# OpenDriveLab/ThinkTwice

Hardware: AMD Instinct MI355X
Metric: frames/sec forward (4-cam+LiDAR, thinktwice.py cfg) (higher is better)
Workload: dtype bf16x3h; 1 GPU; forward_inference thinktwice.py cfg: 8 frames x (2 sweeps x 4 cams x 448x896 + 65536-pt LiDAR), ResNet50+PAFPN+DepthNet+UNet+LSS splat, LidarNet, fusion, 5-stage decoder; parallelism=replicas x1 (no data-path collective), launch=eager launches, 3 batches in flight on alternating streams, batches_in_flight=3

## Files before the change

### include/thinktwice_hip.h

```cpp
#ifndef THINKTWICE_HIP_H
#define THINKTWICE_HIP_H

#include <stddef.h>
#include <stdint.h>

#ifdef __cplusplus
extern "C" {
#endif

#define TT_F32 0
#define TT_BF16 1
#define TT_F16 2

#define TT_ACT_NONE 0
#define TT_ACT_RELU 1
#define TT_ACT_SIGMOID 2
#define TT_ACT_GELU 3
#define TT_ACT_SOFTPLUS 4
#define TT_ACT_SOFTPLUS_CLAMP 5

const char* tt_last_error(void);
const char* tt_conv_last_kernel(void);
int tt_conv_set_trace(void* stamps_or_null);
int tt_version(void);
// ... 124 lines not shown
int tt_mlp_chain_wide_set_max_spin(int polls);
int tt_mlp_chain_wide_set_trace(void* stamps_or_null);

long long tt_dec_gru_scratch_floats(int B);
int tt_dec_gru(int B, const float* inp6, const float* state, float* fut, float* scratch, const void* const* w0,
               const float* const* wx, const float* const* b0, const void* const* w2, const float* const* b2,
               const void* wd0, const float* bd0, const void* wd2, const float* bd2, void* stream);
long long tt_dec_flatten_scratch_floats(int maps);
int tt_dec_flatten(int maps, const float* in, float* out, float* mids_or_null, float* scratch, const void* const* w,
                   const float* const* b, const float* bn_scale, const float* bn_shift, void* stream);
int tt_dec_set_trace(void* stamps_or_null);
long long tt_dec_bev_update_scratch_floats(int B);
int tt_dec_bev_update(int B, const float* bev, const float* G, float* out, long long out_bstride, float* out2,
                      long long out2_bstride, float* scratch, const void* w0, const float* b0, const void* const* w2,
                      const float* b2, void* stream);

int tt_nchw_to_nhwc_pad(const float* in, void* out, int N, int C, int H, int W, int Cp,
                        int out_dtype, void* stream);
int tt_nchw_to_nhwc_border(const float* in, void* out, int N, int C, int H, int W, int Cp, int Hp, int Wp,
                           int top, int left, int out_dtype, void* stream);
int tt_nhwc_to_nchw(const void* in, float* out, int N, int C, int H, int W, int cstride, int coff,
                    int in_dtype, void* stream);
int tt_maxpool3x3s2(const void* in, void* out, int N, int H, int W, int C, int dtype, void* stream);
int tt_upsample_nearest_add(void* dst, const void* src, int N, int H, int W, int C, int h, int w,
                            int dtype, void* stream);
int tt_bilinear_up2(const void* in, void* out, int N, int H, int W, int C, int dtype, void* stream);
int tt_bilinear_up2_pair(const float* in, float* out, int N, int H, int W, int C, void* stream);
int tt_spatial_pool(const void* in, float* out, int N, int HW, int C, int cstride, int coff, int mode,
                    int dtype, void* stream);
int tt_channel_gate(const void* x, const float* gate, const void* res, void* out, int N, int HW, int C,
                    int gate_act, int out_act, int dtype, void* stream);
int tt_affine_rows(const void* x, const float* scale, const float* shift, void* out, long long R, int C,
                   int x_stride, int out_stride, int act, int dtype, void* stream);
int tt_layernorm_rows(const void* x, const float* gamma, const float* beta, void* out, long long R,
                      int D, int x_stride, int out_stride, float eps, int dtype, void* stream);
int tt_copy_nhwc(const void* in, void* out, int N, int H, int W, int C, int in_cstride, int in_coff,
                 int out_cstride, int out_coff, int rot_flip, int in_dtype, int out_dtype, void* stream);
int tt_broadcast_rows(const void* v, void* out, int N, int HW, int C, int v_stride, int out_cstride,
                      int out_coff, int dtype, void* stream);
int tt_ew(const void* a, const void* b, const void* g, void* out, long long R, int C, int a_stride,
          int a_coff, int b_stride, int b_coff, int g_stride, int g_coff, int o_stride, int o_coff,
          int op, int act, int dtype, void* stream);
int tt_concat_rows(float* out, long long R, int out_stride, int nseg, const float* const* srcs, const int* strides,
                   const int* widths, const int* coffs, const int* divs, const int* mods, void* stream);

int tt_deform_im2col3x3(const void* x, const float* offsets, void* cols, int N, int H, int W, int C,
// ... 415 lines not shown
```

### thinktwice_amd/build.py

```python
import os
import subprocess
import sys
from concurrent.futures import ThreadPoolExecutor

from . import _lib

HERE = os.path.dirname(os.path.abspath(__file__))
CSRC = os.path.join(HERE, "csrc")
OBJ = os.path.join(CSRC, "_obj")
LIB = os.path.join(HERE, "libthinktwice_hip.so")
HIPCC = os.environ.get("HIPCC", "/opt/rocm/bin/hipcc")
FLAGS = ["--offload-arch=gfx950", "-O3", "-std=c++17", "-fPIC", "-munsafe-fp-atomics", "-ffp-contract=off",
         "-Wno-unused-result"]


EXTRA_FLAGS = {"conv_x3_pipe.hip": ["-fno-slp-vectorize"], "conv_x3_up2.hip": ["-fno-slp-vectorize"],
               "conv_x3_patch.hip": ["-fno-slp-vectorize"], "conv_x3_join.hip": ["-fno-slp-vectorize"]}


def _sources():
    return sorted(f for f in os.listdir(CSRC) if f.endswith((".hip", ".cpp")))


def _deps_mtime():
    hdrs = [os.path.join(CSRC, f) for f in os.listdir(CSRC) if f.endswith((".h", ".inc"))]
    hdrs.append(os.path.join(HERE, "..", "include", "thinktwice_hip.h"))
    hdrs.append(os.path.abspath(__file__))
    return max(os.path.getmtime(h) for h in hdrs)


def _compile(src, hdr_mtime, verbose):
    obj = os.path.join(OBJ, src + ".o")
    spath = os.path.join(CSRC, src)
    if os.path.exists(obj) and os.path.getmtime(obj) > max(os.path.getmtime(spath), hdr_mtime):
        return obj
    cmd = [HIPCC] + FLAGS + EXTRA_FLAGS.get(src, []) + (["-x", "hip"] if src.endswith(".hip") else []) + ["-c", spath, "-o", obj]
    if verbose:
        print(" ".join(cmd), flush=True)
    subprocess.run(cmd, check=True)
    return obj
# ... 73 lines not shown
```

### thinktwice_amd/csrc/plan_thunks.inc

```

static int thunk_tt_voxel_pool_fwd(const PlanVal* a, void* stream) { return tt_voxel_pool_fwd((int)a[0].i, (int)a[1].i, (int)a[2].i, (int)a[3].i, (int)a[4].i, (int)a[5].i, (const int32_t*)a[6].p, (const float*)a[7].p, (float*)a[8].p, (int32_t*)a[9].p, stream); }
static int thunk_tt_voxel_pool_fwd_ws(const PlanVal* a, void* stream) { return tt_voxel_pool_fwd_ws((int)a[0].i, (int)a[1].i, (int)a[2].i, (int)a[3].i, (int)a[4].i, (int)a[5].i, (const int32_t*)a[6].p, (const float*)a[7].p, (float*)a[8].p, (int32_t*)a[9].p, (void*)a[10].p, (long long)a[11].i, stream); }
static int thunk_tt_voxel_pool_plan_build(const PlanVal* a, void* stream) { return tt_voxel_pool_plan_build((int)a[0].i, (int)a[1].i, (int)a[2].i, (int)a[3].i, (int)a[4].i, (const int32_t*)a[5].p, (void*)a[6].p, (long long)a[7].i, (void*)a[8].p, (long long)a[9].i, stream); }
static int thunk_tt_voxel_pool_fwd_planned(const PlanVal* a, void* stream) { return tt_voxel_pool_fwd_planned((int)a[0].i, (int)a[1].i, (int)a[2].i, (int)a[3].i, (int)a[4].i, (const void*)a[5].p, (const float*)a[6].p, (float*)a[7].p, (void*)a[8].p, (long long)a[9].i, stream); }
static int thunk_tt_voxel_pool_bwd(const PlanVal* a, void* stream) { return tt_voxel_pool_bwd((int)a[0].i, (int)a[1].i, (int)a[2].i, (int)a[3].i, (int)a[4].i, (const int32_t*)a[5].p, (const float*)a[6].p, (float*)a[7].p, stream); }
static int thunk_tt_frustum_voxel_index(const PlanVal* a, void* stream) { return tt_frustum_voxel_index((int)a[0].i, (int)a[1].i, (int)a[2].i, (int)a[3].i, (int)a[4].i, (const float*)a[5].p, (const float*)a[6].p, (const float*)a[7].p, (const float*)a[8].p, (int32_t*)a[9].p, (float*)a[10].p, stream); }
static int thunk_tt_lift_splat_fwd(const PlanVal* a, void* stream) { return tt_lift_splat_fwd((int)a[0].i, (int)a[1].i, (int)a[2].i, (int)a[3].i, (int)a[4].i, (int)a[5].i, (int)a[6].i, (int)a[7].i, (int)a[8].i, (const void*)a[9].p, (const void*)a[10].p, (int)a[11].i, (const int32_t*)a[12].p, (float*)a[13].p, (int)a[14].i, (int)a[15].i, (int)a[16].i, stream); }
static int thunk_tt_lift_splat_fwd_ws(const PlanVal* a, void* stream) { return tt_lift_splat_fwd_ws((int)a[0].i, (int)a[1].i, (int)a[2].i, (int)a[3].i, (int)a[4].i, (int)a[5].i, (int)a[6].i, (int)a[7].i, (int)a[8].i, (const void*)a[9].p, (const void*)a[10].p, (int)a[11].i, (const int32_t*)a[12].p, (float*)a[13].p, (int)a[14].i, (int)a[15].i, (int)a[16].i, (void*)a[17].p, (long long)a[18].i, stream); }
static int thunk_tt_conv2d_fwd(const PlanVal* a, void* stream) { return tt_conv2d_fwd((const tt_conv_desc*)a[0].p, stream); }
static int thunk_tt_conv2d_fwd_next(const PlanVal* a, void* stream) { return tt_conv2d_fwd_next((const tt_conv_desc*)a[0].p, (const tt_conv_next*)a[1].p, stream); }
static int thunk_tt_seg_feedback_chain(const PlanVal* a, void* stream) { return tt_seg_feedback_chain((const float*)a[0].p, (long long)a[1].i, (int)a[2].i, (int)a[3].i, (const float*)a[4].p, (const float*)a[5].p, (const float*)a[6].p, (int)a[7].i, (const float*)a[8].p, (const void*)a[9].p, (int)a[10].i, (const float*)a[11].p, (const float*)a[12].p, (int)a[13].i, (float*)a[14].p, (int)a[15].i, (int)a[16].i, stream); }
static int thunk_tt_mlp_chain(const PlanVal* a, void* stream) { return tt_mlp_chain((const float*)a[0].p, (long long)a[1].i, (int)a[2].i, (int)a[3].i, (const tt_chain_stage*)a[4].p, (int)a[5].i, stream); }
static int thunk_tt_mlp_chain_wide(const PlanVal* a, void* stream) { return tt_mlp_chain_wide((const float*)a[0].p, (long long)a[1].i, (int)a[2].i, (int)a[3].i, (const tt_chain_stage*)a[4].p, (int)a[5].i, (void*)a[6].p, (long long)a[7].i, stream); }
static int thunk_tt_dec_gru(const PlanVal* a, void* stream) { return tt_dec_gru((int)a[0].i, (const float*)a[1].p, (const float*)a[2].p, (float*)a[3].p, (float*)a[4].p, (const void* const*)a[5].p, (const float* const*)a[6].p, (const float* const*)a[7].p, (const void* const*)a[8].p, (const float* const*)a[9].p, (const void*)a[10].p, (const float*)a[11].p, (const void*)a[12].p, (const float*)a[13].p, stream); }
static int thunk_tt_dec_flatten(const PlanVal* a, void* stream) { return tt_dec_flatten((int)a[0].i, (const float*)a[1].p, (float*)a[2].p, (float*)a[3].p, (float*)a[4].p, (const void* const*)a[5].p, (const float* const*)a[6].p, (const float*)a[7].p, (const float*)a[8].p, stream); }
static int thunk_tt_dec_bev_update(const PlanVal* a, void* stream) { return tt_dec_bev_update((int)a[0].i, (const float*)a[1].p, (const float*)a[2].p, (float*)a[3].p, (long long)a[4].i, (float*)a[5].p, (long long)a[6].i, (float*)a[7].p, (const void*)a[8].p, (const float*)a[9].p, (const void* const*)a[10].p, (const float*)a[11].p, stream); }
static int thunk_tt_nchw_to_nhwc_pad(const PlanVal* a, void* stream) { return tt_nchw_to_nhwc_pad((const float*)a[0].p, (void*)a[1].p, (int)a[2].i, (int)a[3].i, (int)a[4].i, (int)a[5].i, (int)a[6].i, (int)a[7].i, stream); }
static int thunk_tt_nchw_to_nhwc_border(const PlanVal* a, void* stream) { return tt_nchw_to_nhwc_border((const float*)a[0].p, (void*)a[1].p, (int)a[2].i, (int)a[3].i, (int)a[4].i, (int)a[5].i, (int)a[6].i, (int)a[7].i, (int)a[8].i, (int)a[9].i, (int)a[10].i, (int)a[11].i, stream); }
static int thunk_tt_nhwc_to_nchw(const PlanVal* a, void* stream) { return tt_nhwc_to_nchw((const void*)a[0].p, (float*)a[1].p, (int)a[2].i, (int)a[3].i, (int)a[4].i, (int)a[5].i, (int)a[6].i, (int)a[7].i, (int)a[8].i, stream); }
static int thunk_tt_maxpool3x3s2(const PlanVal* a, void* stream) { return tt_maxpool3x3s2((const void*)a[0].p, (void*)a[1].p, (int)a[2].i, (int)a[3].i, (int)a[4].i, (int)a[5].i, (int)a[6].i, stream); }
static int thunk_tt_upsample_nearest_add(const PlanVal* a, void* stream) { return tt_upsample_nearest_add((void*)a[0].p, (const void*)a[1].p, (int)a[2].i, (int)a[3].i, (int)a[4].i, (int)a[5].i, (int)a[6].i, (int)a[7].i, (int)a[8].i, stream); }
static int thunk_tt_bilinear_up2(const PlanVal* a, void* stream) { return tt_bilinear_up2((const void*)a[0].p, (void*)a[1].p, (int)a[2].i, (int)a[3].i, (int)a[4].i, (int)a[5].i, (int)a[6].i, stream); }
static int thunk_tt_bilinear_up2_pair(const PlanVal* a, void* stream) { return tt_bilinear_up2_pair((const float*)a[0].p, (float*)a[1].p, (int)a[2].i, (int)a[3].i, (int)a[4].i, (int)a[5].i, stream); }
static int thunk_tt_spatial_pool(const PlanVal* a, void* stream) { return tt_spatial_pool((const void*)a[0].p, (float*)a[1].p, (int)a[2].i, (int)a[3].i, (int)a[4].i, (int)a[5].i, (int)a[6].i, (int)a[7].i, (int)a[8].i, stream); }
static int thunk_tt_channel_gate(const PlanVal* a, void* stream) { return tt_channel_gate((const void*)a[0].p, (const float*)a[1].p, (const void*)a[2].p, (void*)a[3].p, (int)a[4].i, (int)a[5].i, (int)a[6].i, (int)a[7].i, (int)a[8].i, (int)a[9].i, stream); }
static int thunk_tt_affine_rows(const PlanVal* a, void* stream) { return tt_affine_rows((const void*)a[0].p, (const float*)a[1].p, (const float*)a[2].p, (void*)a[3].p, (long long)a[4].i, (int)a[5].i, (int)a[6].i, (int)a[7].i, (int)a[8].i, (int)a[9].i, stream); }
static int thunk_tt_layernorm_rows(const PlanVal* a, void* stream) { return tt_layernorm_rows((const void*)a[0].p, (const float*)a[1].p, (const float*)a[2].p, (void*)a[3].p, (long long)a[4].i, (int)a[5].i, (int)a[6].i, (int)a[7].i, (float)a[8].d, (int)a[9].i, stream); }
static int thunk_tt_copy_nhwc(const PlanVal* a, void* stream) { return tt_copy_nhwc((const void*)a[0].p, (void*)a[1].p, (int)a[2].i, (int)a[3].i, (int)a[4].i, (int)a[5].i, (int)a[6].i, (int)a[7].i, (int)a[8].i, (int)a[9].i, (int)a[10].i, (int)a[11].i, (int)a[12].i, stream); }
static int thunk_tt_broadcast_rows(const PlanVal* a, void* stream) { return tt_broadcast_rows((const void*)a[0].p, (void*)a[1].p, (int)a[2].i, (int)a[3].i, (int)a[4].i, (int)a[5].i, (int)a[6].i, (int)a[7].i, (int)a[8].i, stream); }
static int thunk_tt_ew(const PlanVal* a, void* stream) { return tt_ew((const void*)a[0].p, (const void*)a[1].p, (const void*)a[2].p, (void*)a[3].p, (long long)a[4].i, (int)a[5].i, (int)a[6].i, (int)a[7].i, (int)a[8].i, (int)a[9].i, (int)a[10].i, (int)a[11].i, (int)a[12].i, (int)a[13].i, (int)a[14].i, (int)a[15].i, (int)a[16].i, stream); }
static int thunk_tt_concat_rows(const PlanVal* a, void* stream) { return tt_concat_rows((float*)a[0].p, (long long)a[1].i, (int)a[2].i, (int)a[3].i, (const float* const*)a[4].p, (const int*)a[5].p, (const int*)a[6].p, (const int*)a[7].p, (const int*)a[8].p, (const int*)a[9].p, stream); }
static int thunk_tt_deform_im2col3x3(const PlanVal* a, void* stream) { return tt_deform_im2col3x3((const void*)a[0].p, (const float*)a[1].p, (void*)a[2].p, (int)a[3].i, (int)a[4].i, (int)a[5].i, (int)a[6].i, (int)a[7].i, (int)a[8].i, (int)a[9].i, stream); }
static int thunk_tt_look_project_pack(const PlanVal* a, void* stream) { return tt_look_project_pack((int)a[0].i, (const float*)a[1].p, (const float*)a[2].p, (const float*)a[3].p, (float)a[4].d, (float)a[5].d, (float*)a[6].p, (int*)a[7].p, (int*)a[8].p, (int*)a[9].p, stream); }
static int thunk_tt_look_gather_query(const PlanVal* a, void* stream) { return tt_look_gather_query((int)a[0].i, (const int*)a[1].p, (const float*)a[2].p, (const float*)a[3].p, (const float*)a[4].p, (const float*)a[5].p, (const float*)a[6].p, (const float*)a[7].p, (const float*)a[8].p, (const void* const*)a[9].p, (const int*)a[10].p, (int)a[11].i, (float*)a[12].p, (int)a[13].i, stream); }
static int thunk_tt_msda_sample(const PlanVal* a, void* stream) { return tt_msda_sample((int)a[0].i, (const void*)a[1].p, (int)a[2].i, (const float*)a[3].p, (const float*)a[4].p, (const float*)a[5].p, (const int*)a[6].p, (float*)a[7].p, stream); }
static int thunk_tt_msda_sample_strided(const PlanVal* a, void* stream) { return tt_msda_sample_strided((int)a[0].i, (const void*)a[1].p, (int)a[2].i, (int)a[3].i, (int)a[4].i, (const float*)a[5].p, (const float*)a[6].p, (const float*)a[7].p, (const int*)a[8].p, (float*)a[9].p, stream); }
static int thunk_tt_sca_reduce(const PlanVal* a, void* stream) { return tt_sca_reduce((int)a[0].i, (const float*)a[1].p, (const int*)a[2].p, (float*)a[3].p, stream); }
static int thunk_tt_look_query_ln(const PlanVal* a, void* stream) { return tt_look_query_ln((int)a[0].i, (const int*)a[1].p, (const float*)a[2].p, (const float*)a[3].p, (const float*)a[4].p, (int)a[5].i, (const float*)a[6].p, (const float*)a[7].p, (const float*)a[8].p, (const float*)a[9].p, (const void* const*)a[10].p, (const int*)a[11].p, (int)a[12].i, (const float*)a[13].p, (const float*)a[14].p, (float)a[15].d, (float*)a[16].p, (int)a[17].i, stream); }
static int thunk_tt_msda_sample_ln(const PlanVal* a, void* stream) { return tt_msda_sample_ln((int)a[0].i, (const void*)a[1].p, (int)a[2].i, (int)a[3].i, (int)a[4].i, (const float*)a[5].p, (const float*)a[6].p, (const float*)a[7].p, (const int*)a[8].p, (const float*)a[9].p, (const float*)a[10].p, (float)a[11].d, (float*)a[12].p, (float*)a[13].p, (const int*)a[14].p, stream); }
static int thunk_tt_msda_sample_proj_ln(const PlanVal* a, void* stream) { return tt_msda_sample_proj_ln((int)a[0].i, (const void* const*)a[1].p, (const int*)a[2].p, (const float*)a[3].p, (const float*)a[4].p, (const float*)a[5].p, (const float*)a[6].p, (const float*)a[7].p, (const float*)a[8].p, (const float*)a[9].p, (const float*)a[10].p, (float)a[11].d, (float*)a[12].p, (float*)a[13].p, (const int*)a[14].p, stream); }
static int thunk_tt_sca_reduce_ln(const PlanVal* a, void* stream) { return tt_sca_reduce_ln((int)a[0].i, (const float*)a[1].p, (const int*)a[2].p, (const float*)a[3].p, (const float*)a[4].p, (float)a[5].d, (float*)a[6].p, stream); }
static int thunk_tt_dec_merge_in(const PlanVal* a, void* stream) { return tt_dec_merge_in((int)a[0].i, (const float*)a[1].p, (const float*)a[2].p, (const float*)a[3].p, (const float*)a[4].p, (const float*)a[5].p, (const float*)a[6].p, (float)a[7].d, (float*)a[8].p, stream); }
static int thunk_tt_lidar_voxelize(const PlanVal* a, void* stream) { return tt_lidar_voxelize((const float*)a[0].p, (int)a[1].i, (int)a[2].i, (int)a[3].i, (const float*)a[4].p, (const float*)a[5].p, (const int*)a[6].p, (int)a[7].i, (int)a[8].i, (void*)a[9].p, (long long)a[10].i, (float*)a[11].p, (int*)a[12].p, (int*)a[13].p, stream); }
// ... 65 lines not shown
static int thunk_tt_copy_bytes(const PlanVal* a, void* stream) { return tt_copy_bytes((void*)a[0].p, (const void*)a[1].p, (long long)a[2].i, stream); }

static const PlanThunk kPlanThunks[] = {
    {"tt_voxel_pool_fwd", thunk_tt_voxel_pool_fwd, 10},
    {"tt_voxel_pool_fwd_ws", thunk_tt_voxel_pool_fwd_ws, 12},
    {"tt_voxel_pool_plan_build", thunk_tt_voxel_pool_plan_build, 10},
    {"tt_voxel_pool_fwd_planned", thunk_tt_voxel_pool_fwd_planned, 10},
    {"tt_voxel_pool_bwd", thunk_tt_voxel_pool_bwd, 8},
    {"tt_frustum_voxel_index", thunk_tt_frustum_voxel_index, 11},
    {"tt_lift_splat_fwd", thunk_tt_lift_splat_fwd, 17},
    {"tt_lift_splat_fwd_ws", thunk_tt_lift_splat_fwd_ws, 19},
    {"tt_conv2d_fwd", thunk_tt_conv2d_fwd, 1},
    {"tt_conv2d_fwd_next", thunk_tt_conv2d_fwd_next, 2},
    {"tt_seg_feedback_chain", thunk_tt_seg_feedback_chain, 17},
    {"tt_mlp_chain", thunk_tt_mlp_chain, 6},
    {"tt_mlp_chain_wide", thunk_tt_mlp_chain_wide, 8},
    {"tt_dec_gru", thunk_tt_dec_gru, 14},
    {"tt_dec_flatten", thunk_tt_dec_flatten, 9},
    {"tt_dec_bev_update", thunk_tt_dec_bev_update, 12},
    {"tt_nchw_to_nhwc_pad", thunk_tt_nchw_to_nhwc_pad, 8},
    {"tt_nchw_to_nhwc_border", thunk_tt_nchw_to_nhwc_border, 12},
    {"tt_nhwc_to_nchw", thunk_tt_nhwc_to_nchw, 9},
    {"tt_maxpool3x3s2", thunk_tt_maxpool3x3s2, 7},
    {"tt_upsample_nearest_add", thunk_tt_upsample_nearest_add, 9},
    {"tt_bilinear_up2", thunk_tt_bilinear_up2, 7},
    {"tt_bilinear_up2_pair", thunk_tt_bilinear_up2_pair, 6},
    {"tt_spatial_pool", thunk_tt_spatial_pool, 9},
    {"tt_channel_gate", thunk_tt_channel_gate, 10},
    {"tt_affine_rows", thunk_tt_affine_rows, 10},
    {"tt_layernorm_rows", thunk_tt_layernorm_rows, 10},
    {"tt_copy_nhwc", thunk_tt_copy_nhwc, 13},
    {"tt_broadcast_rows", thunk_tt_broadcast_rows, 9},
    {"tt_ew", thunk_tt_ew, 17},
    {"tt_concat_rows", thunk_tt_concat_rows, 10},
    {"tt_deform_im2col3x3", thunk_tt_deform_im2col3x3, 10},
    {"tt_look_project_pack", thunk_tt_look_project_pack, 10},
    {"tt_look_gather_query", thunk_tt_look_gather_query, 14},
    {"tt_msda_sample", thunk_tt_msda_sample, 8},
    {"tt_msda_sample_strided", thunk_tt_msda_sample_strided, 10},
    {"tt_sca_reduce", thunk_tt_sca_reduce, 4},
    {"tt_look_query_ln", thunk_tt_look_query_ln, 18},
    {"tt_msda_sample_ln", thunk_tt_msda_sample_ln, 15},
    {"tt_msda_sample_proj_ln", thunk_tt_msda_sample_proj_ln, 15},
    {"tt_sca_reduce_ln", thunk_tt_sca_reduce_ln, 7},
    {"tt_dec_merge_in", thunk_tt_dec_merge_in, 9},
    {"tt_lidar_voxelize", thunk_tt_lidar_voxelize, 14},
// ... 68 lines not shown
```

### thinktwice_amd/lss.py

```python
import os

import torch

from . import _lib, camera, layers, ops, weights
from .layers import conv_from_sd, conv_from_weight, deconv2x2_from_sd, linear_from_sd, rows, unrows
from .registry import BACKBONES, NECKS, build_neck


class _ResNet50:

    def __init__(self, sd, p, dtype, device):
        vec = weights.vec_of(dtype)
        self.cin_pad = vec
        self.stem = conv_from_sd(sd, p + ".conv1", dtype, device, bn=p + ".bn1", stride=2, pad=3, act="relu",
                                 cin_pad=vec)
        self.stem_rr, self.stem_rr_x3 = None, None
        if weights.storage_dtype(dtype) != torch.float32:
            w = sd[p + ".conv1.weight"].to(device)
            wr = torch.zeros(w.shape[0], 7, 1, 64, dtype=dtype, device=device)
            wr[:, :, 0, :56] = torch.nn.functional.pad(w.permute(0, 2, 3, 1), (0, 5)).reshape(w.shape[0], 7, 56).to(dtype)
            self.stem_rr = wr.contiguous()
        elif dtype == weights.X3 and os.environ.get("TT_X3_STEM_ROWRUN", "1") == "1":
            w = sd[p + ".conv1.weight"].to(device).float()
            wr = torch.zeros(w.shape[0], 7, 1, 32, dtype=torch.float32, device=device)
            wr[:, :, 0, :28] = torch.nn.functional.pad(w.permute(0, 2, 3, 1), (0, 1)).reshape(w.shape[0], 7, 28)
            self.stem_rr = wr.contiguous()
            self.stem_rr_x3 = weights.split_pairs_x3(self.stem_rr)
        self.blocks = []
        for li, nb in enumerate((3, 4, 6, 3), start=1):
            stage = []
            for b in range(nb):
                q = f"{p}.layer{li}.{b}"
                s = 2 if (b == 0 and li > 1) else 1
                blk = {
                    "c1": conv_from_sd(sd, q + ".conv1", dtype, device, bn=q + ".bn1", act="relu"),
                    "c2": conv_from_sd(sd, q + ".conv2", dtype, device, bn=q + ".bn2", stride=s, pad=1, act="relu"),
                    "c3": conv_from_sd(sd, q + ".conv3", dtype, device, bn=q + ".bn3", act="relu"),
                    "ds": conv_from_sd(sd, q + ".downsample.0", dtype, device, bn=q + ".downsample.1", stride=s)
                    if b == 0 else None,
                }
                stage.append(blk)
            self.blocks.append(stage)

    def stem_border(self):
        return (3, 3, 3, 5) if self.stem_rr is not None else None

    def __call__(self, x, bordered=False):
        if bordered:
            NI, Hp, Wp, _ = x.shape
            if layers.BN_TRAIN:
                z = ops.conv2d(x, self.stem_rr, stride=2, pad=0, act=0, in_cstride=self.cin_pad,
                               out_hw=((Hp - 6) // 2, (Wp - 8) // 2), w_x3=self.stem_rr_x3, out_dtype=torch.float32)
                y = ops.batchnorm_train(z, self.stem.bn, self.stem.act, groups=layers.BN_GROUPS)
            else:
                y = ops.conv2d(x, self.stem_rr, stride=2, pad=0, scale=self.stem.scale, shift=self.stem.shift,
                               act=self.stem.act, in_cstride=self.cin_pad, out_hw=((Hp - 6) // 2, (Wp - 8) // 2),
                               w_x3=self.stem_rr_x3)
        else:
            y = self.stem(x, stop_grad=True)
        x = ops.maxpool3x3s2(y)
        outs = []

        def pair_c1(blk, shape):
            c2 = blk["c2"]
            rows2 = shape[0] * (shape[1] // c2.stride) * (shape[2] // c2.stride)
            return (c2.w_x3 is not None and not layers.BN_TRAIN and
                    ops.pair_ok(min(rows2, shape[0] * shape[1] * shape[2]), c2.w.shape[-1], c2.w.shape[0]))

        from . import autodiff
        flat = [blk for stage in self.blocks for blk in stage]
        last = [len(stage) for stage in self.blocks]
        last = [sum(last[:i + 1]) - 1 for i in range(len(last))]
        y1 = None
        for i, blk in enumerate(flat):
            idt = blk["ds"](x) if blk["ds"] is not None else x
            pr = pair_c1(blk, x.shape)
            if y1 is None:
                y1 = blk["c1"](x, out_pair=pr)
            y = blk["c2"](y1, in_pair=pr)
            c3, nb = blk["c3"], flat[i + 1] if i + 1 < len(flat) else None
            rows = y.shape[0] * y.shape[1] * y.shape[2]
            if (nb is not None and autodiff.TAPE is None and not layers.BN_TRAIN and c3.w_x3 is not None and
                    nb["c1"].w_x3 is not None and pair_c1(nb, y.shape) and
# ... 212 lines not shown
        w3 = sd[s + ".unet_layer0.3.weight"].double()
        wl = sd[s + ".conv_last.weight"].double()[:, :, 0, 0]
        wm = torch.einsum("om,mckl->ockl", wl.to(w3.device), w3).float().contiguous()
        bl = sd.get(s + ".conv_last.bias")
        b3 = sd.get(s + ".unet_layer0.3.bias")
        bm = None if (bl is None and b3 is None) else \
            ((0 if bl is None else bl.double()) + (0 if b3 is None else wl.to(b3.device) @ b3.double())).float()
        fused = {"w.weight": wm}
        if bm is not None:
            fused["w.bias"] = bm
        self.seg_fused = conv_from_sd(fused, "w", dt, dev, pad=1)
        r = p + ".seg_res_to_image_feature"
        self.seg2feat = []
        for idx, (st, pd) in zip((0, 3, 6, 9, 12, 15, 18), ((1, 0), (1, 0), (2, 1), (1, 0), (2, 1), (1, 0), (2, 1))):
            self.seg2feat.append(conv_from_sd(sd, f"{r}.{idx}", dt, dev, bn=f"{r}.{idx + 1}", stride=st, pad=pd,
                                              act="relu", cin_pad=self.seg_cp if idx == 0 else None))
        self.merge = conv_from_sd(sd, p + ".merge_seg_and_image", dt, dev, pad=1)
        if self.queue_len != 1:
            self.bev_merge = conv_from_sd(sd, p + ".bev_multiframe_merge", f32, dev, pad=1)
        self._frustum_dev = self.frustum.to(dev)
        self.loaded = True
        return self

    def _trunk(self, x, bordered=False):
        NI = x.shape[0]
        c = self.backbone(x, bordered=bordered)
        H0, W0 = c[0].shape[1:3]
        dt, dev = self.dtype, x.device
        cat2 = torch.empty(NI, H0, W0, 384, dtype=dt, device=dev)
        cat3 = torch.empty(NI, H0 // 2, W0 // 2, 512, dtype=dt, device=dev)
        cat4 = torch.empty(NI, H0 // 4, W0 // 4, 512, dtype=dt, device=dev)
        outs = self.img_neck(c, targets=[(cat2, 128), (cat3, 256), (cat4, 256), None])
        return (cat2, cat3, cat4, outs[3][0])

    def _fpn_views(self, bufs):
        cat2, cat3, cat4, e4 = bufs
        return [(cat2, 128, 256), (cat3, 256, 256), (cat4, 256, 256), (e4, 0, 256)]

    def _se_gate(self, name, m):
        fc1, fc2, cr, ce = self.se[name]
        return unrows(ce(cr(fc2(fc1(rows(m))))))

    def _depth_net(self, src, mlp_in, T):
        NI, h, w, _ = src.shape
        dev, dt = src.device, self.dtype
        m24 = torch.zeros(mlp_in.shape[0], 24, dtype=torch.float32, device=dev)
        self.bn22(mlp_in, out=m24, running_updates=T)
        x = self.reduce(src)
        dbg = getattr(self, "_dbg", None)
# ... 70 lines not shown
        mats = camera.stack_img_metas(img_metas, num_cams)
        return {"gm": camera.geometry_matrices(mats, -1), "mlp_in": camera.depth_mlp_input(mats),
                "lidar2img": mats["lidar2img"], "ida_mat": mats["ida_mat"]}

    def forward(self, img, img_metas, timestamps=None, is_return_depth=False, channel_last=False, consts=None,
                prev_bev=None):
        if not self.loaded:
            raise _lib.TTError("LSS: load_state_dict() first")
        _lib.require_cuda(img)
        if img.dim() == 5:
            img = img.unsqueeze(1)
        B, T, N, C, H, W = img.shape
        assert T == self.queue_len or (prev_bev is not None and T >= 1), "LSS.queue_len must be set correctly in config!"
        assert (H, W) == self.final_dim
        T_all = self.queue_len
        if prev_bev is not None:
            img = img[:, T - 1:]
            T = 1
        if consts is None:
            consts = {k: v.to(img.device) for k, v in self.host_constants(img_metas, N).items()}
        NI = T * B * N
        from . import autodiff
        border = self.backbone.stem_border() if (H % 2 == 0 and W % 2 == 0 and autodiff.TAPE is None) else None
        if border is not None:
            key = (NI, H, W, str(img.device), int(torch.cuda.current_stream(img.device).cuda_stream))
            x = self._xpad.get(key)
            if x is None:
                x = torch.zeros(NI, H + border[0] + border[2], W + border[1] + border[3], self.backbone.cin_pad,
                                dtype=self.dtype, device=img.device)
                self._xpad[key] = x
        else:
            x = torch.empty(NI, H, W, self.backbone.cin_pad, dtype=self.dtype, device=img.device)
        for s in range(T):
            for b in range(B):
                src = img[b, T - 1 - s].contiguous()
                o = (s * B + b) * N
                if border is not None:
                    ops.nchw_to_nhwc_border(src, x[o:o + N], border[0], border[1])
                else:
                    ops.check(ops.lib().tt_nchw_to_nhwc_pad(ops.ptr(src), ops.ptr(x[o:o + N]), N, C, H, W,
                                                            x.shape[-1], ops.dtype_code(x),
                                                            ops.cur_stream(img.device)), "tt_nchw_to_nhwc_pad")
        with layers.bn_groups(T):
            bufs = self._trunk(x, bordered=border is not None)
            fpn2_buf, fpn2_off, _ = self._fpn_views(bufs)[2]
            src = self.neck_conv(fpn2_buf, in_coff=fpn2_off, cin=256)
            mlp_in = consts["mlp_in"]
            depth, merge_in = self._depth_net(src, mlp_in, T)
            seg = self._seg_net(bufs)
            f, first = seg, 0
            if (ops.SEG_CHAIN and autodiff.TAPE is None and not layers.BN_TRAIN and self.dtype == torch.float32
                    and self.seg2feat[1].w_x3 is not None):
                f, first = ops.seg_feedback_chain(seg, self.seg2feat[0], self.seg2feat[1]), 2
            for i, cv in enumerate(self.seg2feat[first:-1], first):
                f = cv(f, stop_grad=(i == 0))
            self.seg2feat[-1](f, out=merge_in, out_coff=256)
            ctx = self.merge(merge_in, out_dtype=torch.float32)
        geom = self.geometry(consts["gm"], B, N)
        vx, vy, vz = (int(v) for v in self.voxel_num)
        OC = self.output_channels
        bev_cat = torch.zeros(B, vy, vx, OC * T_all, dtype=torch.float32, device=img.device)
        BN = B * N
        for s in range(T):
            ops.lift_splat(depth[s * BN:(s + 1) * BN], ctx[s * BN:(s + 1) * BN], geom, (vx, vy, vz), B, N,
                           out=bev_cat, out_coff=s * OC, record=(s == 0))
        if prev_bev is not None:
            assert T_all == 2 and tuple(prev_bev.shape) == (B, vy, vx, OC), prev_bev.shape
# ... 16 lines not shown
```

### thinktwice_amd/ops.py

```python
import contextlib
import ctypes
import os

import torch

from . import _lib
from ._lib import (TT_BF16, TT_F16, TT_F32, TTError, check, clear_device_faults, cur_stream, device_faults, lib, ptr,
                   raise_on_device_fault, require_cuda)
from . import autodiff


def _active_tape():
    return autodiff.TAPE


def _tape(op, *args):
    tape = _active_tape()
    if tape is not None:
        getattr(tape, op)(*args)


def _st(t):
    return cur_stream(t.device)

# ... 529 lines not shown
    N, C, H, W = x.shape
    out = torch.empty(N, H, W, c_pad, dtype=dtype, device=x.device)
    check(lib().tt_nchw_to_nhwc_pad(ptr(x), ptr(out), N, C, H, W, c_pad, dtype_code(out), _st(x)), "tt_nchw_to_nhwc_pad")
    return out


def nhwc_to_nchw(x, C=None, coff=0):
    require_cuda(x)
    N, H, W, Cs = x.shape
    C = C or Cs
    out = torch.empty(N, C, H, W, dtype=torch.float32, device=x.device)
    check(lib().tt_nhwc_to_nchw(ptr(x), ptr(out), N, C, H, W, Cs, coff, dtype_code(x), _st(x)), "tt_nhwc_to_nchw")
    return out


def maxpool3x3s2(x):
    N, H, W, C = x.shape
    out = torch.empty(N, (H + 2 - 3) // 2 + 1, (W + 2 - 3) // 2 + 1, C, dtype=x.dtype, device=x.device)
    check(lib().tt_maxpool3x3s2(ptr(x), ptr(out), N, H, W, C, dtype_code(x), _st(x)), "tt_maxpool3x3s2")
    _tape("maxpool3x3s2", x, out)
    return out


def upsample_nearest_add_(dst, src):
    N, H, W, C = dst.shape
    check(lib().tt_upsample_nearest_add(ptr(dst), ptr(src), N, H, W, C, src.shape[1],
                                        src.shape[2], dtype_code(dst), _st(dst)), "tt_upsample_nearest_add")
    _tape("upsample_nearest_add_", dst, src)
    return dst


PAIR = os.environ.get("TT_X3_PAIR", "1") != "0"


def pair_ok(rows, cin=32, cout=64, taps=9):
    return (PAIR and _active_tape() is None and rows > 4096 and cin % 32 == 0 and taps * cin >= 64 and
            (8 <= cout <= 32 or cout >= 64))


BNECK_JOIN = os.environ.get("TT_BNECK_JOIN", "1") != "0"
JOIN_MIN_ROWS = 32768
JOIN_ROUTED = ((64, 256, 64), (64, 256, 128), (128, 512, 128))


def join_ok(rows, k1, cout, next_cout):
    return BNECK_JOIN and _active_tape() is None and rows >= JOIN_MIN_ROWS and (k1, cout, next_cout) in JOIN_ROUTED
# ... 617 lines not shown
```

Baseline: 114.0 frames/s.

## Fuse image layout conversion, 7x7 stem conv and maxpool into one persistent kernel

Adds a persistent HIP kernel that reads the raw NCHW f32 camera images directly, splits each pixel into bf16 hi/lo parts in LDS, runs the 7x7 stride-2 stem conv as bf16x3 MFMA with fused BN+ReLU, then max-pools 3x3 s2 in LDS and writes the pooled NHWC output. It replaces the per-(s,b) NCHW-to-NHWC padded copies, the stem conv launch and the separate maxpool, removing the full-resolution stem activation round trip through HBM. The kernel uses a halo-tiled scheme with duplicated halo conv work, double-buffered patch loads, and is limited to the f32 inference path with a grid capped at the CU count.

Measured after the change: 116.1 frames/s, median of 6. +1.9%, better.

```diff
diff --git a/include/thinktwice_hip.h b/include/thinktwice_hip.h
--- a/include/thinktwice_hip.h
+++ b/include/thinktwice_hip.h
@@ -170,6 +170,10 @@
 int tt_nhwc_to_nchw(const void* in, float* out, int N, int C, int H, int W, int cstride, int coff,
                     int in_dtype, void* stream);
 int tt_maxpool3x3s2(const void* in, void* out, int N, int H, int W, int C, int dtype, void* stream);
+int tt_stem_pool_x3(const float* img, long long stride_b, long long stride_t, long long stride_n, long long stride_c,
+                    long long stride_h, long long stride_w, int B, int T, int N, int H, int W, int img_dtype,
+                    const void* weight_x3, int w_cout, int w_kh, int w_k, const float* scale, const float* shift,
+                    float* out, long long out_floats, int max_workgroups, void* stream);
 int tt_upsample_nearest_add(void* dst, const void* src, int N, int H, int W, int C, int h, int w,
                             int dtype, void* stream);
 int tt_bilinear_up2(const void* in, void* out, int N, int H, int W, int C, int dtype, void* stream);
diff --git a/thinktwice_amd/build.py b/thinktwice_amd/build.py
--- a/thinktwice_amd/build.py
+++ b/thinktwice_amd/build.py
@@ -15,7 +15,8 @@
 
 
 EXTRA_FLAGS = {"conv_x3_pipe.hip": ["-fno-slp-vectorize"], "conv_x3_up2.hip": ["-fno-slp-vectorize"],
-               "conv_x3_patch.hip": ["-fno-slp-vectorize"], "conv_x3_join.hip": ["-fno-slp-vectorize"]}
+               "conv_x3_patch.hip": ["-fno-slp-vectorize"], "conv_x3_join.hip": ["-fno-slp-vectorize"],
+               "conv_x3_stem.hip": ["-fno-slp-vectorize"]}
 
 
 def _sources():
diff --git a/thinktwice_amd/csrc/conv_x3_stem.hip b/thinktwice_amd/csrc/conv_x3_stem.hip
--- /dev/null
+++ b/thinktwice_amd/csrc/conv_x3_stem.hip
@@ -0,0 +1,243 @@
+#include "conv_common.h"
+
+namespace tt {
+namespace {
+
+constexpr int kPH = 7, kPW = 8;
+constexpr int kSH = 2 * kPH + 1, kSW = 2 * kPW + 1;
+constexpr int kRows = kSH * kSW;
+constexpr int kIH = 2 * kSH + 5, kIW = 2 * kSW + 6;
+constexpr int kInPix = kIH * kIW;
+constexpr int kInHalf = kInPix * 8;
+constexpr int kLdc = 72;
+constexpr int kStemBytes = 256 * kLdc * 4;
+constexpr int kThreads = 512;
+constexpr int kInPerThread = (kInPix + kThreads - 1) / kThreads;
+constexpr int kPoolTasks = kPH * kPW * 16;
+constexpr int kPoolPerThread = (kPoolTasks + kThreads - 1) / kThreads;
+constexpr size_t kStemLds = 2 * (size_t)kInHalf + kStemBytes;
+static_assert(kRows <= 256 && kRows > 224, "eight 32-row blocks");
+
+struct StemPoolArgs {
+    const float* img;
+    long long sb, st, sn;
+    int B, T, N, H, W;
+    int SH, SW, PH, PW;
+    int tiles_y, tiles_x, ntiles;
+    const float* w;
+    const float* scale;
+    const float* shift;
+    float* out;
+};
+
+}
+
+__global__ __launch_bounds__(kThreads) void conv_x3_stem_pool_kernel(const StemPoolArgs p) {
+#if defined(__HIP_DEVICE_COMPILE__)
+    extern __shared__ __attribute__((aligned(16))) unsigned char smem[];
+    unsigned char* const in_hi = smem;
+    float* const stem = reinterpret_cast<float*>(smem + 2 * kInHalf);
+    const int tid = threadIdx.x, lane = tid & 63;
+    const int wave = __builtin_amdgcn_readfirstlane(tid >> 6);
+    const int r = lane & 31, half = lane >> 5;
+    const int nb = wave & 1;
+    const int mb0 = (wave >> 1) * 2;
+
+    uint4 bh[14], bl[14];
+    {
+        const float* wrow = p.w + (long long)(nb * 32 + r) * (7 * 32);
+#pragma unroll
+        for (int ks = 0; ks < 14; ++ks) {
+            bh[ks] = *reinterpret_cast<const uint4*>(wrow + ks * 16 + half * 4);
+            bl[ks] = *reinterpret_cast<const uint4*>(wrow + ks * 16 + 8 + half * 4);
+        }
+    }
+    const float sc = p.scale[nb * 32 + r], sh = p.shift[nb * 32 + r];
+
+    unsigned a_off[2];
+#pragma unroll
+    for (int i = 0; i < 2; ++i) {
+        int m = (mb0 + i) * 32 + r;
+        m = m < kRows ? m : kRows - 1;
+        const int sy = m / kSW, sx = m - sy * kSW;
+        a_off[i] = (unsigned)(((2 * sy) * kIW + 2 * sx + 2 * half) * 8);
+    }
+
+    const int grid = (int)gridDim.x;
+    const int slot = (int)blockIdx.x;
+    const int tiles_per_img = p.tiles_y * p.tiles_x;
+    const long long plane = (long long)p.H * p.W;
+
+    float px[kInPerThread][3];
+    unsigned px_ok = 0;
+    auto load_patch = [&](int tile) {
+        const int i = tile / tiles_per_img, rem = tile - i * tiles_per_img;
+        const int ty = rem / p.tiles_x, tx = rem - ty * p.tiles_x;
+        const int s = i / (p.B * p.N), bn = i - s * (p.B * p.N);
+        const int b = bn / p.N, n = bn - b * p.N;
+        const float* src = p.img + b * p.sb + (long long)(p.T - 1 - s) * p.st + n * p.sn;
+        const int iy0 = 4 * kPH * ty - 5, ix0 = 4 * kPW * tx - 5;
+        px_ok = 0;
+#pragma unroll
+        for (int k = 0; k < kInPerThread; ++k) {
+            const int q = tid + k * kThreads;
+            const int row = q / kIW, col = q - row * kIW;
+            const int y = iy0 + row, x = ix0 + col;
+            const bool ok = q < kInPix && y >= 0 && y < p.H && x >= 0 && x < p.W;
+            const float* g = src + (long long)(ok ? y : 0) * p.W + (ok ? x : 0);
+            px_ok |= ok ? 1u << k : 0u;
+#pragma unroll
+            for (int c = 0; c < 3; ++c) px[k][c] = g[c * plane];
+        }
+    };
+    auto store_patch = [&]() {
+#pragma unroll
+        for (int k = 0; k < kInPerThread; ++k) {
+            const int q = tid + k * kThreads;
+            if (q < kInPix) {
+                const bool ok = (px_ok >> k) & 1u;
+                const float x[4] = {ok ? px[k][0] : 0.f, ok ? px[k][1] : 0.f, ok ? px[k][2] : 0.f, 0.f};
+                uint32_t h[2], l[2];
+#pragma unroll
+                for (int e = 0; e < 2; ++e) {
+                    h[e] = pack_bf16x2(x[2 * e], x[2 * e + 1]);
+                    l[e] = pack_bf16x2(x[2 * e] - hi0_f32(h[e]), x[2 * e + 1] - hi1_f32(h[e]));
+                }
+                *reinterpret_cast<uint2*>(in_hi + q * 8) = make_uint2(h[0], h[1]);
+                *reinterpret_cast<uint2*>(in_hi + kInHalf + q * 8) = make_uint2(l[0], l[1]);
+            }
+        }
+    };
+
+    int tile = slot;
+    if (tile < p.ntiles) load_patch(tile);
+#pragma unroll
+    for (int ks = 0; ks < 14; ++ks) {
+        asm volatile("" ::"v"(bh[ks].x), "v"(bl[ks].x));
+    }
+    if (tile < p.ntiles) store_patch();
+    while (tile < p.ntiles) {
+        __syncthreads();
+        const int next = tile + grid;
+        if (next < p.ntiles) load_patch(next);
+
+        f32x16 acc[2];
+        zero_acc(acc);
+#pragma unroll
+        for (int ks = 0; ks < 14; ++ks) {
+            const unsigned o = (unsigned)((ks >> 1) * (kIW * 8) + (ks & 1) * 32);
+            uint4 ah[2], al[2];
+#pragma unroll
+            for (int i = 0; i < 2; ++i) {
+                ah[i] = *reinterpret_cast<const uint4*>(in_hi + a_off[i] + o);
+                al[i] = *reinterpret_cast<const uint4*>(in_hi + kInHalf + a_off[i] + o);
+            }
+            Mfma<uint16_t>::run(al[0], bh[ks], acc[0]);
+            Mfma<uint16_t>::run(al[1], bh[ks], acc[1]);
+            Mfma<uint16_t>::run(ah[0], bl[ks], acc[0]);
+            Mfma<uint16_t>::run(ah[1], bl[ks], acc[1]);
+            Mfma<uint16_t>::run(ah[0], bh[ks], acc[0]);
+            Mfma<uint16_t>::run(ah[1], bh[ks], acc[1]);
+        }
+
+#pragma unroll
+        for (int i = 0; i < 2; ++i)
+#pragma unroll
+            for (int e = 0; e < 16; ++e) {
+                const int row = (mb0 + i) * 32 + (e & 3) + 8 * (e >> 2) + 4 * half;
+                const float v = acc[i][e] * sc + sh;
+                stem[row * kLdc + nb * 32 + r] = v > 0.f ? v : 0.f;
+            }
+        __syncthreads();
+        if (next < p.ntiles) store_patch();
+
+        {
+            const int i = tile / tiles_per_img, rem = tile - i * tiles_per_img;
+            const int ty = rem / p.tiles_x, tx = rem - ty * p.tiles_x;
+            const int py0 = kPH * ty, px0 = kPW * tx;
+            const int sy0 = 2 * py0 - 1, sx0 = 2 * px0 - 1;
+            typedef float f4v __attribute__((ext_vector_type(4)));
+#pragma unroll
+            for (int k = 0; k < kPoolPerThread; ++k) {
+                const int q = tid + k * kThreads;
+                const int pp = q >> 4, cg = q & 15;
+                const int pyl = pp >> 3, pxl = pp & 7;
+                const int py = py0 + pyl, pxg = px0 + pxl;
+                float4 v[9];
+#pragma unroll
+                for (int dy = 0; dy < 3; ++dy) {
+                    const int sg = sy0 + 2 * pyl + dy;
+                    const int sl = (sg < 0 || sg >= p.SH) ? 2 * pyl + 1 : 2 * pyl + dy;
+#pragma unroll
+                    for (int dx = 0; dx < 3; ++dx) {
+                        const int cgl = sx0 + 2 * pxl + dx;
+                        const int cl = (cgl < 0 || cgl >= p.SW) ? 2 * pxl + 1 : 2 * pxl + dx;
+                        v[dy * 3 + dx] = *reinterpret_cast<const float4*>(stem + (sl * kSW + cl) * kLdc + cg * 4);
+                    }
+                }
+                float m[4] = {-INFINITY, -INFINITY, -INFINITY, -INFINITY};
+#pragma unroll
+                for (int e = 0; e < 9; ++e) {
+                    m[0] = fmaxf(m[0], v[e].x);
+                    m[1] = fmaxf(m[1], v[e].y);
+                    m[2] = fmaxf(m[2], v[e].z);
+                    m[3] = fmaxf(m[3], v[e].w);
+                }
+                if (q < kPoolTasks && py < p.PH && pxg < p.PW) {
+                    float* o = p.out + (((long long)i * p.PH + py) * p.PW + pxg) * 64 + cg * 4;
+                    __builtin_nontemporal_store(f4v{m[0], m[1], m[2], m[3]}, reinterpret_cast<f4v*>(o));
+                }
+            }
+        }
+        tile = next;
+    }
+#endif
+}
+
+}
+
+extern "C" int tt_stem_pool_x3(const float* img, long long stride_b, long long stride_t, long long stride_n, long long stride_c,
+                               long long stride_h, long long stride_w, int B, int T, int N, int H, int W, int img_dtype,
+                               const void* weight_x3, int w_cout, int w_kh, int w_k, const float* scale, const float* shift,
+                               float* out, long long out_floats, int max_workgroups, void* stream) {
+    using namespace tt;
+    TT_REQUIRE(img_dtype == TT_F32, "tt_stem_pool_x3: img_dtype=%d: f32 storage only (the 16-bit stems keep their three launches)", img_dtype);
+    TT_REQUIRE(img && out, "tt_stem_pool_x3: img / out is null");
+    TT_REQUIRE(B > 0 && T > 0 && N > 0 && H > 0 && W > 0, "tt_stem_pool_x3: B=%d T=%d N=%d H=%d W=%d must be positive", B, T, N, H, W);
+    TT_REQUIRE(H % 2 == 0, "tt_stem_pool_x3: H=%d must be even", H);
+    TT_REQUIRE(W % 2 == 0, "tt_stem_pool_x3: W=%d must be even", W);
+    TT_REQUIRE(stride_w == 1 && stride_h == W && stride_c == (long long)H * W,
+               "tt_stem_pool_x3: stride_c=%lld stride_h=%lld stride_w=%lld: the inner (3, H, W) block must be contiguous", stride_c,
+               stride_h, stride_w);
+    TT_REQUIRE(stride_b >= 0 && stride_t >= 0 && stride_n >= 0, "tt_stem_pool_x3: stride_b / stride_t / stride_n must not be negative");
+    TT_REQUIRE(weight_x3, "tt_stem_pool_x3: weight_x3 is null");
+    TT_REQUIRE(w_cout == 64 && w_kh == 7 && w_k == 32, "tt_stem_pool_x3: weight_x3 shape [%d][%d][1][%d]: the row-run stem is [64][7][1][32]",
+               w_cout, w_kh, w_k);
+    TT_REQUIRE(((uintptr_t)weight_x3 & 15) == 0, "tt_stem_pool_x3: weight_x3 must be 16-byte aligned");
+    TT_REQUIRE(scale && shift, "tt_stem_pool_x3: scale / shift is null");
+    TT_REQUIRE(((uintptr_t)out & 15) == 0, "tt_stem_pool_x3: out must be 16-byte aligned");
+    const long long NI = (long long)B * T * N;
+    const int SH = H / 2, SW = W / 2, PH = (SH + 1) / 2, PW = (SW + 1) / 2;
+    TT_REQUIRE(out_floats >= NI * PH * PW * 64, "tt_stem_pool_x3: out_floats=%lld is too small for (%lld, %d, %d, 64)", out_floats, NI, PH,
+               PW);
+    TT_REQUIRE(max_workgroups >= 0, "tt_stem_pool_x3: max_workgroups=%d must not be negative", max_workgroups);
+    StemPoolArgs a;
+    a.img = img;
+    a.sb = stride_b; a.st = stride_t; a.sn = stride_n;
+    a.B = B; a.T = T; a.N = N; a.H = H; a.W = W;
+    a.SH = SH; a.SW = SW; a.PH = PH; a.PW = PW;
+    a.tiles_y = div_up(PH, kPH);
+    a.tiles_x = div_up(PW, kPW);
+    const long long ntiles = NI * a.tiles_y * a.tiles_x;
+    TT_REQUIRE(ntiles < (1ll << 31) && (long long)H * W < (1ll << 31), "tt_stem_pool_x3: %lld tiles / %d x %d pixels overflow an int", ntiles, H, W);
+    a.ntiles = (int)ntiles;
+    a.w = reinterpret_cast<const float*>(weight_x3);
+    a.scale = scale;
+    a.shift = shift;
+    a.out = out;
+    if (lds_opt_in(reinterpret_cast<const void*>(conv_x3_stem_pool_kernel), kStemLds, "tt_stem_pool_x3")) return -1;
+    int grid = (int)(ntiles < kNumCU ? ntiles : kNumCU);
+    if (max_workgroups > 0 && max_workgroups < grid) grid = max_workgroups;
+    hipLaunchKernelGGL(conv_x3_stem_pool_kernel, dim3((unsigned)grid), dim3(kThreads), kStemLds, (hipStream_t)stream, a);
+    return check_launch("tt_stem_pool_x3");
+}
diff --git a/thinktwice_amd/csrc/plan_thunks.inc b/thinktwice_amd/csrc/plan_thunks.inc
--- a/thinktwice_amd/csrc/plan_thunks.inc
+++ b/thinktwice_amd/csrc/plan_thunks.inc
@@ -19,6 +19,7 @@
 static int thunk_tt_nchw_to_nhwc_border(const PlanVal* a, void* stream) { return tt_nchw_to_nhwc_border((const float*)a[0].p, (void*)a[1].p, (int)a[2].i, (int)a[3].i, (int)a[4].i, (int)a[5].i, (int)a[6].i, (int)a[7].i, (int)a[8].i, (int)a[9].i, (int)a[10].i, (int)a[11].i, stream); }
 static int thunk_tt_nhwc_to_nchw(const PlanVal* a, void* stream) { return tt_nhwc_to_nchw((const void*)a[0].p, (float*)a[1].p, (int)a[2].i, (int)a[3].i, (int)a[4].i, (int)a[5].i, (int)a[6].i, (int)a[7].i, (int)a[8].i, stream); }
 static int thunk_tt_maxpool3x3s2(const PlanVal* a, void* stream) { return tt_maxpool3x3s2((const void*)a[0].p, (void*)a[1].p, (int)a[2].i, (int)a[3].i, (int)a[4].i, (int)a[5].i, (int)a[6].i, stream); }
+static int thunk_tt_stem_pool_x3(const PlanVal* a, void* stream) { return tt_stem_pool_x3((const float*)a[0].p, (long long)a[1].i, (long long)a[2].i, (long long)a[3].i, (long long)a[4].i, (long long)a[5].i, (long long)a[6].i, (int)a[7].i, (int)a[8].i, (int)a[9].i, (int)a[10].i, (int)a[11].i, (int)a[12].i, (const void*)a[13].p, (int)a[14].i, (int)a[15].i, (int)a[16].i, (const float*)a[17].p, (const float*)a[18].p, (float*)a[19].p, (long long)a[20].i, (int)a[21].i, stream); }
 static int thunk_tt_upsample_nearest_add(const PlanVal* a, void* stream) { return tt_upsample_nearest_add((void*)a[0].p, (const void*)a[1].p, (int)a[2].i, (int)a[3].i, (int)a[4].i, (int)a[5].i, (int)a[6].i, (int)a[7].i, (int)a[8].i, stream); }
 static int thunk_tt_bilinear_up2(const PlanVal* a, void* stream) { return tt_bilinear_up2((const void*)a[0].p, (void*)a[1].p, (int)a[2].i, (int)a[3].i, (int)a[4].i, (int)a[5].i, (int)a[6].i, stream); }
 static int thunk_tt_bilinear_up2_pair(const PlanVal* a, void* stream) { return tt_bilinear_up2_pair((const float*)a[0].p, (float*)a[1].p, (int)a[2].i, (int)a[3].i, (int)a[4].i, (int)a[5].i, stream); }
@@ -130,6 +131,7 @@
     {"tt_nchw_to_nhwc_border", thunk_tt_nchw_to_nhwc_border, 12},
     {"tt_nhwc_to_nchw", thunk_tt_nhwc_to_nchw, 9},
     {"tt_maxpool3x3s2", thunk_tt_maxpool3x3s2, 7},
+    {"tt_stem_pool_x3", thunk_tt_stem_pool_x3, 22},
     {"tt_upsample_nearest_add", thunk_tt_upsample_nearest_add, 9},
     {"tt_bilinear_up2", thunk_tt_bilinear_up2, 7},
     {"tt_bilinear_up2_pair", thunk_tt_bilinear_up2_pair, 6},
diff --git a/thinktwice_amd/lss.py b/thinktwice_amd/lss.py
--- a/thinktwice_amd/lss.py
+++ b/thinktwice_amd/lss.py
@@ -45,8 +45,13 @@
     def stem_border(self):
         return (3, 3, 3, 5) if self.stem_rr is not None else None
 
-    def __call__(self, x, bordered=False):
-        if bordered:
+    def stem_pool_ok(self, img):
+        return self.stem_rr_x3 is not None and ops.stem_pool_ok(img, self.stem_rr_x3)
+
+    def __call__(self, x, bordered=False, image=False):
+        if image:
+            x = ops.stem_pool(x, self.stem_rr_x3, self.stem.scale, self.stem.shift)
+        elif bordered:
             NI, Hp, Wp, _ = x.shape
             if layers.BN_TRAIN:
                 z = ops.conv2d(x, self.stem_rr, stride=2, pad=0, act=0, in_cstride=self.cin_pad,
@@ -58,7 +63,8 @@
                                w_x3=self.stem_rr_x3)
         else:
             y = self.stem(x, stop_grad=True)
-        x = ops.maxpool3x3s2(y)
+        if not image:
+            x = ops.maxpool3x3s2(y)
         outs = []
 
         def pair_c1(blk, shape):
@@ -317,9 +323,9 @@
         self.loaded = True
         return self
 
-    def _trunk(self, x, bordered=False):
-        NI = x.shape[0]
-        c = self.backbone(x, bordered=bordered)
+    def _trunk(self, x, bordered=False, image=False):
+        NI = x.shape[0] * x.shape[1] * x.shape[2] if image else x.shape[0]
+        c = self.backbone(x, bordered=bordered, image=image)
         H0, W0 = c[0].shape[1:3]
         dt, dev = self.dtype, x.device
         cat2 = torch.empty(NI, H0, W0, 384, dtype=dt, device=dev)
@@ -436,7 +442,10 @@
         NI = T * B * N
         from . import autodiff
         border = self.backbone.stem_border() if (H % 2 == 0 and W % 2 == 0 and autodiff.TAPE is None) else None
-        if border is not None:
+        fused_stem = border is not None and self.backbone.stem_pool_ok(img)
+        if fused_stem:
+            x = img
+        elif border is not None:
             key = (NI, H, W, str(img.device), int(torch.cuda.current_stream(img.device).cuda_stream))
             x = self._xpad.get(key)
             if x is None:
@@ -445,7 +454,7 @@
                 self._xpad[key] = x
         else:
             x = torch.empty(NI, H, W, self.backbone.cin_pad, dtype=self.dtype, device=img.device)
-        for s in range(T):
+        for s in range(0 if fused_stem else T):
             for b in range(B):
                 src = img[b, T - 1 - s].contiguous()
                 o = (s * B + b) * N
@@ -456,7 +465,7 @@
                                                             x.shape[-1], ops.dtype_code(x),
                                                             ops.cur_stream(img.device)), "tt_nchw_to_nhwc_pad")
         with layers.bn_groups(T):
-            bufs = self._trunk(x, bordered=border is not None)
+            bufs = self._trunk(x, bordered=border is not None, image=fused_stem)
             fpn2_buf, fpn2_off, _ = self._fpn_views(bufs)[2]
             src = self.neck_conv(fpn2_buf, in_coff=fpn2_off, cin=256)
             mlp_in = consts["mlp_in"]
diff --git a/thinktwice_amd/ops.py b/thinktwice_amd/ops.py
--- a/thinktwice_amd/ops.py
+++ b/thinktwice_amd/ops.py
@@ -575,6 +575,35 @@
     return out
 
 
+STEM_POOL = os.environ.get("TT_STEM_POOL", "1") != "0"
+
+
+def stem_pool_ok(img, w_x3):
+    from . import layers
+    if not (STEM_POOL and _active_tape() is None and not layers.BN_TRAIN and w_x3 is not None and img.dtype == torch.float32 and
+            img.dim() == 6 and img.shape[3] == 3 and img.shape[4] % 2 == 0 and img.shape[5] % 2 == 0):
+        return False
+    B, T, N, _, H, W = img.shape
+    return tuple(img.stride()[3:]) == (H * W, W, 1) and B * T * N * (H // 2) * (W // 2) > 4096
+
+
+def stem_pool(img, w_x3, scale, shift, max_workgroups=0):
+    require_cuda(img, w_x3, scale, shift)
+    B, T, N, C, H, W = img.shape
+    NI, PH, PW = B * T * N, (H // 2 + 1) // 2, (W // 2 + 1) // 2
+    out = torch.empty(NI, PH, PW, 64, dtype=torch.float32, device=img.device)
+    sb, st, sn, sc, sh, sw = img.stride()
+    with _launch() as rec:
+        check(lib().tt_stem_pool_x3(ptr(img), sb, st, sn, sc, sh, sw, B, T, N, H, W, dtype_code(img), ptr(w_x3), w_x3.shape[0],
+                                    w_x3.shape[1], w_x3.shape[-1], ptr(scale), ptr(shift), ptr(out), out.numel(), max_workgroups,
+                                    _st(img)), "tt_stem_pool_x3")
+    if rec is not None:
+        M = NI * (H // 2) * (W // 2)
+        rec.log(2.0 * M * 64 * 224, f"M={M} N=64 K=224 stem+pool k7x7s2", kernel="conv_x3_stem_pool_kernel",
+                nbytes=NI * 3 * H * W * 4 + out.numel() * 4 + w_x3.numel() * 4)
+    return out
+
+
 def upsample_nearest_add_(dst, src):
     N, H, W, C = dst.shape
     check(lib().tt_upsample_nearest_add(ptr(dst), ptr(src), N, H, W, C, src.shape[1],
```
